# gongaa/Feedback-GNN

Measured on AMD Instinct MI355X. Metric: decoded codewords/sec, [[882,24]] 64-iter BP4 + feedback-GNN, higher is better.
Workload: dtype f32

## Files before the change

feedback_gnn_amd/csrc/fgnn_bp4.hip:

```cpp

#include <type_traits>

#include "fgnn_internal.h"
#include "fgnn_math.h"
#include "fgnn_math_ranged.h"
#include "fgnn_cn.h"

#ifndef FGNN_BP4_WAVES
#define FGNN_BP4_WAVES 7
#endif
#ifndef FGNN_HWT_PIN_CLIP_POINTS
#define FGNN_HWT_PIN_CLIP_POINTS 1
#endif
#ifndef FGNN_PHI_STAGE
#define FGNN_PHI_STAGE 1
#endif

namespace {

struct BpArgs {
    int B, num_iter, tpc, cpb, lds_per_cw, lch_off;
    float factor, llr_const;
    const float* llr_ch;
    const uint8_t* synd_x;
// ... 46 lines not shown
    {
        const float y = exp(-FG_MIN(FG_ABS(a - b), 20.0f));
        return log(1.0f + y);
    }
    static __device__ __forceinline__ float lse2(float a, float b)
    {
        return lse2_corr(a, b) + FG_MAX(a, b);
    }
    static __device__ __forceinline__ float phi(float x)
    {
        const float xc = FG_CLAMP(x, FG_PHI_MIN, FG_PHI_MAX);
        const float y = exp(xc);
        const float sp = (xc > FG_SOFTPLUS_THRESH) ? xc : log(1.0f + y);
        float r = sp - log(y - 1.0f);
#if FGNN_HWT_PIN_CLIP_POINTS
        r = (x >= FG_PHI_MAX) ? 0.0f : r;
        r = (x <= FG_PHI_MIN) ? 16.6355324f : r;
#endif
        return r;
    }
};

template <bool HWT = false>
__device__ __forceinline__ float logit_row_opt(const float* llr, const int* __restrict__ col, int deg, float phi0, bool shortcut)
{
    if (shortcut) {
        unsigned neg = 0;
        bool sat = true;
        for (int j = 0; j < deg; ++j) {
            const float v = llr[col[j]];
            neg ^= (v < 0.0f);
            sat = sat && (FG_ABS(v) >= FG_PHI_MAX);
        }
        if (__all(sat)) return with_sign(phi0, neg);
    }
    return logit_row<Mx<HWT>>(llr, col, deg);
}

template <int N, bool HWT = false>
__device__ __forceinline__ void phi_n(const float (&x)[N], float (&out)[N])
{
    if constexpr (HWT) {
#pragma unroll
        for (int k = 0; k < N; ++k) out[k] = Mx<true>::phi(x[k]);
        return;
    }
    const float* tab = fg_log_tab();
    float xc[N], y[N];
    uint32_t eb1[N], eb2[N], j1[N], j2[N];
#pragma unroll
    for (int k = 0; k < N; ++k) {
        xc[k] = FG_CLAMP(x[k], FG_PHI_MIN, FG_PHI_MAX);
        y[k] = fg_exp(xc[k]);
        const uint32_t w1 = fg_f2u(1.0f + y[k]) - FG_LOG_OFFS;
        const uint32_t w2 = fg_f2u(y[k] - 1.0f) - FG_LOG_OFFS;
        eb1[k] = w1 & 0xff800000u;
        eb2[k] = w2 & 0xff800000u;
        j1[k] = (w1 >> 18) & 31u;
        j2[k] = (w2 >> 18) & 31u;
    }
    __builtin_amdgcn_sched_barrier(0);
    float rc1[N], lc1[N], rc2[N], lc2[N];
#pragma unroll
    for (int k = 0; k < N; ++k) {
        rc1[k] = tab[j1[k]];
        lc1[k] = tab[32 + j1[k]];
        rc2[k] = tab[j2[k]];
        lc2[k] = tab[32 + j2[k]];
    }
    __builtin_amdgcn_sched_barrier(0);
#pragma unroll
    for (int k = 0; k < N; ++k) {
        const float a = fg_u2f(fg_f2u(rc1[k]) - eb1[k]);
        const float r1 = FG_FMA(y[k], a, a - 1.0f);
        float sp = FG_FMA((float)(int32_t)eb1[k], FG_LN2_S23, lc1[k] + fg_log1p_small(r1));
        sp = (xc[k] > FG_SOFTPLUS_THRESH) ? xc[k] : sp;
        const float mm = fg_u2f(fg_f2u(y[k] - 1.0f) - eb2[k]);
        const float r2 = FG_FMA(mm, rc2[k], -1.0f);
        const float lg = FG_FMA((float)(int32_t)eb2[k], FG_LN2_S23, lc2[k] + fg_log1p_small(r2));
        out[k] = sp - lg;
    }
}

template <int DC, bool HWT = false, bool F1 = false>
__device__ __forceinline__ bool cn_phi_regular(float* msg, const int (&sl)[DC], uint32_t neg0, float factor, float phi0,
                                               bool shortcut)
{
    constexpr int H = (DC % FGNN_PHI_STAGE == 0) ? FGNN_PHI_STAGE : DC / 2;
    static_assert(DC % H == 0, "a phi stage must take a whole fraction of a check");
    float v[DC], aa[DC];
    uint32_t neg = neg0;
    bool sat = true;
#pragma unroll
    for (int j = 0; j < DC; ++j) {
        v[j] = slot_ref(msg, sl[j]);
        neg ^= fg_f2u(v[j]);
        sat = sat && (FG_ABS(v[j]) >= FG_PHI_MAX);
    }
    if (shortcut && __all(sat)) {
#pragma unroll
        for (int j = 0; j < DC; ++j) {
            const float o = fg_u2f(fg_f2u(phi0) | ((neg ^ fg_f2u(v[j])) & 0x80000000u));
            slot_ref(msg, sl[j]) = F1 ? o : o * factor;
        }
        return true;
    }
#pragma unroll
    for (int g0 = 0; g0 < DC; g0 += H) {
        float xa[H], oa[H];
#pragma unroll
        for (int j = 0; j < H; ++j) xa[j] = FG_ABS(v[g0 + j]);
        phi_n<H, HWT>(xa, oa);
#pragma unroll
        for (int j = 0; j < H; ++j) aa[g0 + j] = oa[j];
    }
    float T = 0.0f;
#pragma unroll
    for (int j = 0; j < DC; ++j) T = T + aa[j];
#pragma unroll
    for (int g0 = 0; g0 < DC; g0 += H) {
        float xa[H], oa[H];
#pragma unroll
        for (int j = 0; j < H; ++j) xa[j] = T - aa[g0 + j];
        phi_n<H, HWT>(xa, oa);
#pragma unroll
        for (int j = 0; j < H; ++j) {
            const float o = fg_u2f(fg_f2u(oa[j]) | ((neg ^ fg_f2u(v[g0 + j])) & 0x80000000u));
            slot_ref(msg, sl[g0 + j]) = F1 ? o : o * factor;
        }
    }
    return false;
}

template <int DC>
__device__ __forceinline__ void cn_tanh_regular(float* msg, const int (&sl)[DC], unsigned synd, float factor)
{
    float t[DC];
    float P = 1.0f;
#pragma unroll
    for (int j = 0; j < DC; ++j) {
        float tj = fg_tanh(slot_ref(msg, sl[j]) / 2.0f);
        tj = (tj == 0.0f) ? 1e-12f : tj;
        P = (j == 0) ? tj : P * tj;
        t[j] = tj;
    }
    P = P * (synd ? -1.0f : 1.0f);
    const float clipv = 0.99999988f;
#pragma unroll
    for (int j = 0; j < DC; ++j) {
        float q = fg_rcp_unit(t[j]) * P;
        q = (FG_ABS(q) < 1e-7f) ? 0.0f : q;
        q = FG_MIN(FG_MAX(q, -clipv), clipv);
        slot_ref(msg, sl[j]) = (2.0f * fg_atanh(q)) * factor;
    }
}

template <bool HWT = false>
__device__ __forceinline__ bool cn_phi_generic(float* msg, const int* __restrict__ slot, int deg, unsigned synd, float factor,
                                               float phi0, bool shortcut)
{
    if (shortcut) {
        unsigned neg = synd;
        bool sat = true;
        for (int j = 0; j < deg; ++j) {
            const float v = msg[slot[j]];
            neg ^= (v < 0.0f);
            sat = sat && (FG_ABS(v) >= FG_PHI_MAX);
        }
        if (__all(sat)) {
            for (int j = 0; j < deg; ++j) {
                const int s = slot[j];
                msg[s] = with_sign(phi0, neg ^ (unsigned)(msg[s] < 0.0f)) * factor;
            }
            return true;
        }
    }
    cn_update<FGNN_CN_BOXPLUS_PHI, Mx<HWT>>(msg, slot, deg, synd, factor);
    return false;
}

__device__ __forceinline__ float softplus_saturated(float t)
{
    const float y = fg_exp(FG_MIN(FG_MAX(t, -87.0f), 0.0f));
    return (t > 0.0f) ? t : ((t < -87.0f) ? 0.0f : y);
}

template <int CN_TYPE, int DVX, int DVZ, int DC, bool OPT, bool HWT = false, int NQ = 0, bool TRACE = false, bool GMEM = false, int LSE = 2,
          int NT = 0>
__global__ void __launch_bounds__(1024) __attribute__((amdgpu_waves_per_eu(NQ > 0 ? FGNN_BP4_WAVES - 1 : FGNN_BP4_WAVES)))
bp4_kernel(GraphDev g, BpArgs a)
{
    static_assert(!(HWT && OPT), "the hardware-transcendental variant is the fixed dataflow only: the exact shortcuts are proofs about fgnn_math.h");
    static_assert(!GMEM || (DVX == 0 && !OPT && !HWT && NQ == 0 && !TRACE), "the global-memory variant is the plain runtime-degree kernel");
    using MX = Mx<HWT>;
    FG_LOG_TAB_SETUP();
    constexpr bool REGULAR = DVX > 0;
    constexpr bool LREG = NQ > 0;
    constexpr int NQA = LREG ? NQ : 1;
    static_assert(NT == 0 || (DVX > 0 && CN_TYPE == FGNN_CN_BOXPLUS_PHI && !LREG && !TRACE && !GMEM), "compile-time trips: the regular phi kernel");
    constexpr int CT = LREG ? NQ : NT;
    const int tpc = NT > 0 ? 256 : a.tpc;
    const bool opt_shortcut = OPT && a.shortcut != 0;
    const bool opt_exit = OPT && a.early_exit != 0;
    const bool shl = LSE == 2 ? a.shared_lse != 0 : LSE == 1;
    extern __shared__ float lds[];
    const int cwl = NT > 0 ? 0 : threadIdx.x / tpc;
    const int lane = threadIdx.x - cwl * tpc;
    const int slot_b = NT > 0 ? blockIdx.x : blockIdx.x * a.cpb + cwl;
    const bool active = slot_b < a.B;
    const int b = (active && a.index) ? a.index[slot_b] : slot_b;
    float* msg;
    if constexpr (GMEM) msg = a.gmem + (size_t)slot_b * a.lds_per_cw;
    else if constexpr (NT > 0) msg = lds;
    else msg = lds + (size_t)cwl * a.lds_per_cw;
    float* Lch = msg + a.lch_off;
    const int n = g.n;

    constexpr bool CLOSED_OK = REGULAR && CN_TYPE == FGNN_CN_BOXPLUS_PHI && !LREG && !TRACE;
    const bool zero_start = REGULAR && !TRACE && !a.msg_init_x && !a.msg_init_z && a.num_iter > 0;
    const bool first_closed = CLOSED_OK && zero_start && !a.llr_ch;
    const bool first_peeled = zero_start && a.llr_ch != nullptr;
    const bool fill = !first_closed && !first_peeled;
    if (active) {
        if (fill) {
            for (int e = lane; e < g.E_x; e += tpc) msg[e] = a.msg_init_x ? a.msg_init_x[(size_t)b * g.E_x + e] : 0.0f;
            for (int e = lane; e < g.E_z; e += tpc)
                msg[g.E_x + e] = a.msg_init_z ? a.msg_init_z[(size_t)b * g.E_z + e] : 0.0f;
        }
        if (a.llr_ch && !LREG)
            for (int i = lane; i < 3 * n; i += tpc) Lch[i] = a.llr_ch[(size_t)b * 3 * n + i];
    }
    float lreg[3][NQA];
    if constexpr (LREG) {
#pragma unroll
        for (int i = 0; i < NQ; ++i) {
            const int v = lane + i * tpc;
            const bool in = active && v < n;
#pragma unroll
            for (int c = 0; c < 3; ++c) lreg[c][i] = in ? a.llr_ch[(size_t)b * 3 * n + c * n + v] : 0.0f;
        }
    }
    if (fill || (a.llr_ch && !LREG)) __syncthreads();

    const uint8_t* sx = a.synd_x + (size_t)b * g.m_x;
    const uint8_t* sz = a.synd_z + (size_t)b * g.m_z;
    const int lane_c = lane + (tpc >> 1) < tpc ? lane + (tpc >> 1) : lane - tpc + (tpc >> 1);

    const float phi0 = MX::phi(0.0f);
    (void)phi0;
    unsigned* sigw = reinterpret_cast<unsigned*>(msg + a.sig_off);
    int* flags = reinterpret_cast<int*>(sigw + n);
    bool a1 = false, a2 = false;
    if (opt_exit) {
        for (int v = lane; v < n; v += tpc) sigw[v] = fill ? 0xffffffffu : 0u;
        if (lane < 4) flags[lane] = 0;
        __syncthreads();
    }
    int it_begin = 0;
    if constexpr (CLOSED_OK) {
        if (first_closed) {
            const float L = a.llr_const;
            const float Y = (0.0f + 0.0f) + L, X = 0.0f + L, Z = 0.0f + L;
            const float nu_x = MX::softplus(-X) - MX::lse2(-(Z - 0.0f), -(Y - 0.0f));
            const float nu_z = MX::softplus(-Z) - MX::lse2(-(X - 0.0f), -(Y - 0.0f));
            if (active)
                for (int c = lane_c; c < g.m; c += tpc) {
                    const unsigned synd = (c < g.m_x ? sx[c] : sz[c - g.m_x]) & 1u;
                    const uint4 pk = reinterpret_cast<const uint4*>(g.cslot16)[c];
                    const unsigned w[4] = {pk.x, pk.y, pk.z, pk.w};
                    const float nu = c < g.m_x ? nu_x : nu_z;
                    const unsigned ng = nu < 0.0f;
                    unsigned neg = synd;
                    const float aa = MX::phi(FG_ABS(nu));
                    float T = 0.0f;
#pragma unroll
                    for (int j = 0; j < DC; ++j) {
                        neg ^= ng;
                        T = T + aa;
                    }
                    const float val = with_sign(MX::phi(T - aa), neg ^ ng) * a.factor;
#pragma unroll
                    for (int j = 0; j < DC; ++j) slot_ref(msg, (int)((w[j >> 1] >> ((j & 1) * 16)) & 0xffffu)) = val;
                }
            if (opt_exit) a1 = FG_ABS(nu_x) >= FG_PHI_MAX && FG_ABS(nu_z) >= FG_PHI_MAX;
            it_begin = 1;
            __syncthreads();
        }
    }
    const bool cn_one = a.cpb == 1, cn_f1 = a.factor == 1.0f;
    unsigned synd_bits = 0;
    if (active) {
        int i = 0;
        for (int c = lane_c; c < g.m && i < 32; c += tpc, ++i) synd_bits |= ((c < g.m_x ? sx[c] : sz[c - g.m_x]) & 1u) << i;
    }
    const bool synd_in_reg = (g.m + tpc - 1) / tpc <= 32;
    unsigned row_off = 16u * (unsigned)lane_c;
    auto trace_step = [&](const int k) __attribute__((always_inline)) {
        float* tlx = msg + a.trace_off;
        float* tlz = tlx + n;
        if (active && a.tape_x) {
            float* px = a.tape_x + ((size_t)k * a.B + b) * g.E_x;
            float* pz = a.tape_z + ((size_t)k * a.B + b) * g.E_z;
            for (int e = lane; e < g.E_x; e += tpc) px[e] = msg[e];
            for (int e = lane; e < g.E_z; e += tpc) pz[e] = msg[g.E_x + e];
        }
        if (active)
            for (int v = lane; v < n; v += tpc) {
                const int x0 = g.vptr_x[v], x1 = g.vptr_x[v + 1], z0 = g.vptr_z[v], z1 = g.vptr_z[v + 1];
                float Sz = 0.0f, Sx = 0.0f;
                for (int e = z0; e < z1; ++e) Sz = Sz + msg[e];
                for (int e = x0; e < x1; ++e) Sx = Sx + msg[e];
                const float lx = a.llr_ch ? Lch[v] : a.llr_const, ly = a.llr_ch ? Lch[n + v] : a.llr_const,
                            lz = a.llr_ch ? Lch[2 * n + v] : a.llr_const;
                const float Y = (Sz + Sx) + ly;
                const float X = Sz + lx;
                const float Z = Sx + lz;
                tlz[v] = MX::softplus(-X) - MX::lse2(-Z, -Y);
                tlx[v] = MX::softplus(-Z) - MX::lse2(-X, -Y);
            }
        __syncthreads();
        if (active) {
            float* tx = a.trace_x + ((size_t)k * a.B + b) * g.rows[0];
            for (int r = lane; r < g.rows[0]; r += tpc) {
                const int p0 = g.rptr[0][r];
                tx[r] = logit_row<Mx<HWT>>(tlx, g.rcol[0] + p0, g.rptr[0][r + 1] - p0);
            }
            float* tz = a.trace_z + ((size_t)k * a.B + b) * g.rows[1];
            for (int r = lane; r < g.rows[1]; r += tpc) {
                const int p0 = g.rptr[1][r];
                tz[r] = logit_row<Mx<HWT>>(tlz, g.rcol[1] + p0, g.rptr[1][r + 1] - p0);
            }
        }
    };
    if constexpr (TRACE) trace_step(0);
    if constexpr (REGULAR && !TRACE) {
        if (first_peeled && active) {
            auto vn_first = [&](const int v, const float lx, const float ly, const float lz) __attribute__((always_inline)) {
                const float Y = (0.0f + 0.0f) + ly;
                const float X = 0.0f + lx;
                const float Z = 0.0f + lz;
                const float numx = MX::softplus(-X);
                const float numz = MX::softplus(-Z);
                const float Ze = Z - 0.0f, Xe = X - 0.0f, Ye = Y - 0.0f;
                float ox, oz;
                if (shl) {
                    ox = numx - (MX::lse2_corr(-Z, -Y) + FG_MAX(-Ze, -Ye));
                    oz = numz - (MX::lse2_corr(-X, -Y) + FG_MAX(-Xe, -Ye));
                } else {
                    ox = numx - MX::lse2(-Ze, -Ye);
                    oz = numz - MX::lse2(-Xe, -Ye);
                }
                float* px = msg + v * DVX;
                float* pz = msg + g.E_x + v * DVZ;
#pragma unroll
                for (int k = 0; k < DVX; ++k) px[k] = ox;
#pragma unroll
                for (int k = 0; k < DVZ; ++k) pz[k] = oz;
            };
            if constexpr (LREG) {
#pragma unroll
                for (int i = 0; i < NQ; ++i) {
                    const int v = lane + i * tpc;
                    if (v < n) vn_first(v, lreg[0][i], lreg[1][i], lreg[2][i]);
                }
            } else {
                for (int v = lane; v < n; v += tpc) vn_first(v, Lch[v], Lch[n + v], Lch[2 * n + v]);
            }
        }
    }
    for (int it = it_begin; it < a.num_iter; ++it) {
        bool changed = false, cn_slow = false;
        auto vn_body = [&](const int v, const float lx, const float ly, const float lz) __attribute__((always_inline)) {
                if constexpr (REGULAR) {
                    float* px = msg + v * DVX;
                    float* pz = msg + g.E_x + v * DVZ;
                    float mx[DVX], mz[DVZ];
                    float Sz = 0.0f, Sx = 0.0f;
#pragma unroll
                    for (int k = 0; k < DVZ; ++k) { mz[k] = pz[k]; Sz = Sz + mz[k]; }
// ... 81 lines not shown
                            sig |= sign_bit(mm) << (e - x0);
                        }
                        for (int e = z0; e < z1; ++e) {
                            const float mm = msg[e];
                            sat = sat && (shl || FG_ABS((X - mm) - (Y - mm)) >= 20.0f);
                            sig |= sign_bit(mm) << ((x1 - x0) + (e - z0));
                        }
                        if (opt_exit && sigw[v] != sig) {
                            changed = true;
                            sigw[v] = sig;
                        }
                        if (__all(sat)) {
                            const float nx = softplus_saturated(-X), nz = softplus_saturated(-Z);
                            for (int e = x0; e < x1; ++e) {
                                const float mm = msg[e];
                                const float Ze = Z - mm, Ye = Y - mm;
                                msg[e] = nx - (0.0f + FG_MAX(-Ze, -Ye));
                            }
                            for (int e = z0; e < z1; ++e) {
                                const float mm = msg[e];
                                const float Xe = X - mm, Ye = Y - mm;
                                msg[e] = nz - (0.0f + FG_MAX(-Xe, -Ye));
                            }
                            return;
                        }
                    }
                    const float numx = MX::softplus(-X);
                    const float numz = MX::softplus(-Z);
                    if (shl) {
                        const float cx = MX::lse2_corr(-Z, -Y), cz = MX::lse2_corr(-X, -Y);
                        for (int e = x0; e < x1; ++e) {
                            float m = msg[e];
                            float Ze = Z - m, Ye = Y - m;
                            msg[e] = numx - (cx + FG_MAX(-Ze, -Ye));
                        }
                        for (int e = z0; e < z1; ++e) {
                            float m = msg[e];
                            float Xe = X - m, Ye = Y - m;
                            msg[e] = numz - (cz + FG_MAX(-Xe, -Ye));
                        }
                        return;
                    }
                    for (int e = x0; e < x1; ++e) {
                        float m = msg[e];
                        float Ze = Z - m, Ye = Y - m;
                        msg[e] = numx - MX::lse2(-Ze, -Ye);
                    }
                    for (int e = z0; e < z1; ++e) {
                        float m = msg[e];
                        float Xe = X - m, Ye = Y - m;
                        msg[e] = numz - MX::lse2(-Xe, -Ye);
                    }
                }
            };
        if (active && !(first_peeled && it == 0)) {
            if constexpr (LREG) {
#pragma unroll
                for (int i = 0; i < NQ; ++i) {
                    const int v = lane + i * tpc;
                    if (v < n) vn_body(v, lreg[0][i], lreg[1][i], lreg[2][i]);
                }
            } else if constexpr (NT > 0) {
#pragma unroll
                for (int i = 0; i < NT; ++i) {
                    const int v = lane + i * 256;
                    if (i + 1 < NT || v < n) vn_body(v, a.llr_const, a.llr_const, a.llr_const);
                }
            } else {
                for (int v = lane; v < n; v += tpc) {
                    if (a.llr_ch) vn_body(v, Lch[v], Lch[n + v], Lch[2 * n + v]);
                    else vn_body(v, a.llr_const, a.llr_const, a.llr_const);
                }
            }
        }
        if (opt_exit && changed) flags[2 * (it & 1)] = 1;
        __syncthreads();
        if (opt_exit && lane == 0) {
            flags[2 * ((it + 1) & 1)] = 0;
            flags[2 * ((it + 1) & 1) + 1] = 0;
        }
        if constexpr (REGULAR && CT > 0 && CN_TYPE == FGNN_CN_BOXPLUS_PHI) {
            auto cn_trips = [&](auto f1) __attribute__((always_inline)) {
                constexpr bool F1 = decltype(f1)::value;
                const char* rows = reinterpret_cast<const char*>(g.cslot16);
#pragma unroll
                for (int i = 0; i < CT; ++i) {
                    const bool in = (!LREG && i + 1 < CT) || lane_c + i * tpc < g.m;
                    if (in) {
                        const char* base = rows + (size_t)i * (size_t)(16u * (unsigned)tpc);
                        asm volatile("" : "+v"(row_off));
                        if constexpr (NT > 0) asm volatile("" : "+s"(base));
                        typedef unsigned Row __attribute__((ext_vector_type(4)));
                        const Row pk = *(const __attribute__((address_space(1))) Row*)(base + row_off);
                        const unsigned w[4] = {pk.x, pk.y, pk.z, pk.w};
                        int sl[DC];
#pragma unroll
                        for (int j = 0; j < DC; ++j) sl[j] = (int)((w[j >> 1] >> ((j & 1) * 16)) & 0xffffu);
                        const bool fast = cn_phi_regular<DC, HWT, F1>(lds, sl, synd_bits << (31 - i), F1 ? 1.0f : a.factor, phi0, opt_shortcut);
                        cn_slow = !fast || cn_slow;
                    }
                }
            };
            if (active) {
                if (cn_f1) cn_trips(std::true_type{});
                else cn_trips(std::false_type{});
            }
        } else if (active) {
            int ci = 0;
            for (int c = lane_c; c < g.m; c += tpc, ++ci) {
                const unsigned synd = synd_in_reg ? (synd_bits >> ci) & 1u : (c < g.m_x ? sx[c] : sz[c - g.m_x]) & 1u;
                if constexpr (REGULAR) {
                    const uint4 pk = reinterpret_cast<const uint4*>(g.cslot16)[c];
                    const unsigned w[4] = {pk.x, pk.y, pk.z, pk.w};
                    int sl[DC];
#pragma unroll
                    for (int j = 0; j < DC; ++j) sl[j] = (int)((w[j >> 1] >> ((j & 1) * 16)) & 0xffffu);
                    if constexpr (CN_TYPE == FGNN_CN_BOXPLUS_PHI) {
                        bool fast;
                        if (cn_one && cn_f1) fast = cn_phi_regular<DC, HWT, true>(lds, sl, synd << 31, 1.0f, phi0, opt_shortcut);
                        else if (cn_one) fast = cn_phi_regular<DC, HWT, false>(lds, sl, synd << 31, a.factor, phi0, opt_shortcut);
                        else fast = cn_phi_regular<DC, HWT, false>(msg, sl, synd << 31, a.factor, phi0, opt_shortcut);
                        cn_slow = !fast || cn_slow;
                    } else if constexpr (CN_TYPE == FGNN_CN_MINSUM) {
                        cn_minsum_regular<DC>(msg, sl, DC, synd, a.factor);
                    } else {
                        cn_tanh_regular<DC>(msg, sl, synd, a.factor);
                    }
                } else {
                    const int c0 = g.cptr[c], deg = g.cptr[c + 1] - c0;
                    if constexpr (CN_TYPE == FGNN_CN_BOXPLUS_PHI)
                        cn_slow = !cn_phi_generic<HWT>(msg, g.cslot + c0, deg, synd, a.factor, phi0, opt_shortcut) || cn_slow;
                    else cn_update<CN_TYPE, Mx<HWT>>(msg, g.cslot + c0, deg, synd, a.factor);
                }
            }
        }
        if (opt_exit && cn_slow) flags[2 * (it & 1) + 1] = 1;
        __syncthreads();
        if (opt_exit) {
            const bool stable = a1 && a2 && flags[2 * (it & 1)] == 0;
            a2 = a1;
            a1 = flags[2 * (it & 1) + 1] == 0;
            if (stable) break;
        }
        if constexpr (TRACE) trace_step(it + 1);
    }

    if (active) {
        if (a.msg_out_x)
            for (int e = lane; e < g.E_x; e += tpc) a.msg_out_x[(size_t)b * g.E_x + e] = msg[e];
        if (a.msg_out_z)
            for (int e = lane; e < g.E_z; e += tpc) a.msg_out_z[(size_t)b * g.E_z + e] = msg[g.E_x + e];
    }
    auto total_body = [&](const int v, const float lx, const float ly, const float lz) __attribute__((always_inline)) {
            const int x0 = g.vptr_x[v], x1 = g.vptr_x[v + 1], z0 = g.vptr_z[v], z1 = g.vptr_z[v + 1];
            float Sz = 0.0f, Sx = 0.0f;
            for (int e = z0; e < z1; ++e) Sz = Sz + msg[e];
            for (int e = x0; e < x1; ++e) Sx = Sx + msg[e];
            const float Y = (Sz + Sx) + ly;
            const float X = Sz + lx;
            const float Z = Sx + lz;
            float* o = a.llr_out + (size_t)b * 3 * n;
            o[v] = X;
            o[n + v] = Y;
            o[2 * n + v] = Z;
            int d = 0;
            float best = 0.0f;
            if (X < best) { best = X; d = 1; }
            if (Z < best) { best = Z; d = 2; }
            if (Y < best) { best = Y; d = 3; }
            a.x_hat[(size_t)b * n + v] = (uint8_t)(d & 1);
            a.z_hat[(size_t)b * n + v] = (uint8_t)(d >> 1);
    };
    if (active) {
        if constexpr (LREG) {
#pragma unroll
            for (int i = 0; i < NQ; ++i) {
                const int v = lane + i * tpc;
                if (v < n) total_body(v, lreg[0][i], lreg[1][i], lreg[2][i]);
            }
        } else {
            for (int v = lane; v < n; v += tpc) {
                if (a.llr_ch) total_body(v, Lch[v], Lch[n + v], Lch[2 * n + v]);
                else total_body(v, a.llr_const, a.llr_const, a.llr_const);
            }
        }
    }
    if (a.flagged) {
        uint8_t* dec = reinterpret_cast<uint8_t*>(msg + a.flag_off);
        unsigned* fword = reinterpret_cast<unsigned*>(dec + ((n + 3) & ~3));
        __syncthreads();
        if (active)
            for (int v = lane; v < n; v += tpc) {
                dec[v] = (uint8_t)(a.x_hat[(size_t)b * n + v] | (a.z_hat[(size_t)b * n + v] << 1));
            }
        if (lane == 0) *fword = 0u;
        __syncthreads();
        unsigned mine = 0;
        if (active)
            for (int c = lane; c < g.m; c += tpc) {
                const int sh = c < g.m_x ? 1 : 0;
                unsigned par = (c < g.m_x ? sx[c] : sz[c - g.m_x]) & 1u;
                for (int e = g.cptr[c]; e < g.cptr[c + 1]; ++e) par ^= (dec[g.cvn[e]] >> sh) & 1u;
                mine |= par;
            }
        if (mine) atomicOr(fword, 1u);
        __syncthreads();
        if (active && lane == 0) a.flagged[b] = (uint8_t)(*fword != 0u);
    }
    if (!a.x_logit && !a.z_logit) return;
    __syncthreads();
    float* llx = msg;
    float* llz = msg + n;
    if (active)
        for (int v = lane; v < n; v += tpc) {
            const float* o = a.llr_out + (size_t)b * 3 * n;
            const float X = o[v], Y = o[n + v], Z = o[2 * n + v];
            const bool sat = opt_shortcut && FG_ABS(X) > FG_SOFTPLUS_THRESH && FG_ABS(Z) > FG_SOFTPLUS_THRESH &&
                             FG_ABS((-Z) - (-Y)) >= 20.0f && FG_ABS((-X) - (-Y)) >= 20.0f;
            if (opt_shortcut && __all(sat)) {
                llz[v] = softplus_saturated(-X) - (0.0f + FG_MAX(-Z, -Y));
                llx[v] = softplus_saturated(-Z) - (0.0f + FG_MAX(-X, -Y));
                continue;
            }
            llz[v] = MX::softplus(-X) - MX::lse2(-Z, -Y);
            llx[v] = MX::softplus(-Z) - MX::lse2(-X, -Y);
        }
    __syncthreads();
    if (active) {
        if (a.x_logit)
            for (int r = lane; r < g.rows[0]; r += tpc) {
                const int p0 = g.rptr[0][r];
                a.x_logit[(size_t)b * g.rows[0] + r] = logit_row_opt<HWT>(llx, g.rcol[0] + p0, g.rptr[0][r + 1] - p0, phi0, opt_shortcut);
            }
        if (a.z_logit)
            for (int r = lane; r < g.rows[1]; r += tpc) {
                const int p0 = g.rptr[1][r];
                a.z_logit[(size_t)b * g.rows[1] + r] = logit_row_opt<HWT>(llz, g.rcol[1] + p0, g.rptr[1][r + 1] - p0, phi0, opt_shortcut);
            }
    }
}

using Bp4Kernel = void (*)(GraphDev, BpArgs);

template <int NQ, bool OPT, int LSE, int NT = 0>
constexpr Bp4Kernel bp4_lse_kernel = bp4_kernel<FGNN_CN_BOXPLUS_PHI, 3, 3, 6, OPT, false, NQ, false, false, LSE, NT>;
constexpr Bp4Kernel bp4_lse_kernels[3][2][2] = {
    {{bp4_lse_kernel<0, false, 0>, bp4_lse_kernel<0, false, 1>}, {bp4_lse_kernel<0, true, 0>, bp4_lse_kernel<0, true, 1>}},
    {{bp4_lse_kernel<4, false, 0>, bp4_lse_kernel<4, false, 1>}, {bp4_lse_kernel<4, true, 0>, bp4_lse_kernel<4, true, 1>}},
    {{bp4_lse_kernel<5, false, 0>, bp4_lse_kernel<5, false, 1>}, {bp4_lse_kernel<5, true, 0>, bp4_lse_kernel<5, true, 1>}}};

constexpr Bp4Kernel bp4_nt_kernels[2][2][2] = {
    {{bp4_lse_kernel<0, false, 0, 4>, bp4_lse_kernel<0, false, 1, 4>}, {bp4_lse_kernel<0, true, 0, 4>, bp4_lse_kernel<0, true, 1, 4>}},
    {{bp4_lse_kernel<0, false, 0, 5>, bp4_lse_kernel<0, false, 1, 5>}, {bp4_lse_kernel<0, true, 0, 5>, bp4_lse_kernel<0, true, 1, 5>}}};

template <int CN_TYPE, int DVX, int DVZ, int DC>
int launch_bp4_k(const fgnn_graph* g, const BpArgs& a, const LaunchGeom& L, size_t lds_bytes, hipStream_t st)
{
    Bp4Kernel kern = a.shortcut ? bp4_kernel<CN_TYPE, DVX, DVZ, DC, true> : bp4_kernel<CN_TYPE, DVX, DVZ, DC, false>;
    if constexpr ((DVX == 3 && DVZ == 3 && DC == 6) || DVX == 0) {
        if (a.trace_x) kern = bp4_kernel<CN_TYPE, DVX, DVZ, DC, false, false, 0, true>;
    }
    if constexpr (CN_TYPE == FGNN_CN_BOXPLUS_PHI) {
        if (a.hwt) kern = bp4_kernel<CN_TYPE, DVX, DVZ, DC, false, true>;
        if constexpr (DVX == 3 && DVZ == 3 && DC == 6) {
            if (!a.trace_x && !a.hwt) kern = bp4_lse_kernels[a.lreg ? a.lreg - 3 : 0][a.shortcut][a.shared_lse];
            if (!a.trace_x && !a.hwt && a.nt) kern = bp4_nt_kernels[a.nt - 4][a.shortcut][a.shared_lse];
        }
    }
    return fgnn_launch(kern, dim3(L.blocks), dim3(L.threads), lds_bytes, st, g->d, a);
}

struct Bp4Plan {
    size_t lds_bytes;
    bool gmem;
    size_t ws_bytes;
};

template <int CN_TYPE>
int launch_bp4(const fgnn_graph* g, const BpArgs& a, const LaunchGeom& L, const Bp4Plan& p, hipStream_t st)
{
    if (p.gmem)
        return fgnn_launch(bp4_kernel<CN_TYPE, 0, 0, 0, false, false, 0, false, true>, dim3(L.blocks), dim3(L.threads), 0, st, g->d, a);
    const GraphDev& d = g->d;
    if (d.cslot16 && !g->force_generic) {
        if (d.dvx == 3 && d.dvz == 3 && d.dc == 6) return launch_bp4_k<CN_TYPE, 3, 3, 6>(g, a, L, p.lds_bytes, st);
        if (d.dvx == 4 && d.dvz == 4 && d.dc == 8 && !a.trace_x) return launch_bp4_k<CN_TYPE, 4, 4, 8>(g, a, L, p.lds_bytes, st);
    }
    return launch_bp4_k<CN_TYPE, 0, 0, 0>(g, a, L, p.lds_bytes, st);
}

Bp4Plan plan_bp4(const fgnn_graph* g, int cn_type, const LaunchGeom& L, BpArgs& a, bool gmem = false)
{
    const GraphDev& d = g->d;
    const int n = d.n;
    const bool trace = a.trace_x != nullptr, phi = cn_type == FGNN_CN_BOXPLUS_PHI;
    auto round4 = [](int floats) { return (floats + 3) & ~3; };
    a.shared_lse = g->bp4_shared_lse ? 1 : 0;
    a.hwt = (g->hw_transcendentals && phi && !trace && !gmem) ? 1 : 0;
    a.shortcut = (g->shortcut && !a.hwt && !trace && !gmem) ? 1 : 0;
    a.lch_off = d.E > 2 * n ? d.E : 2 * n;
    const int per_thread = (n + L.tpc - 1) / L.tpc, per_thread_c = (d.m + L.tpc - 1) / L.tpc;
    const int trips = per_thread > per_thread_c ? per_thread : per_thread_c;
    const bool r336 = d.cslot16 && !g->force_generic && d.dvx == 3 && d.dvz == 3 && d.dc == 6;
    const bool fixed_trips = !trace && !a.hwt && !gmem && phi && L.cpb == 1 && r336;
    a.lreg = (a.llr_ch && fixed_trips && trips <= 5) ? (trips <= 4 ? 4 : 5) : 0;
    a.nt = (!a.llr_ch && fixed_trips && L.tpc == 256 && per_thread == per_thread_c && (trips == 4 || trips == 5)) ? trips : 0;
    int per = a.lch_off + ((a.llr_ch && !a.lreg) ? 3 * n : 0);
    a.trace_off = 0;
    if (trace) {
        a.trace_off = per;
        per += 2 * n;
    }
    if (!gmem) per = round4(per);
    a.sig_off = per;
    int tail = 0;
    a.early_exit = (a.shortcut && g->early_exit && d.max_vdeg <= 32 && phi && L.cpb == 1 && a.num_iter > 2) ? 1 : 0;
    if (a.early_exit) {
        if (((size_t)per * L.cpb + n + 4) * sizeof(float) <= FGNN_LDS_BUDGET) tail += n + 4;
        else a.early_exit = 0;
    }
    a.flag_off = 0;
    if (a.flagged) {
        const int need = round4(n) / 4 + 1;
        if (a.lch_off >= 2 * n + need) {
            a.flag_off = 2 * n;
        } else {
            a.flag_off = per + tail;
            tail += need;
        }
    }
    if (gmem) {
        a.lds_per_cw = round4(per + tail);
        return {0, true, (size_t)L.blocks * (size_t)a.lds_per_cw * sizeof(float)};
    }
    a.lds_per_cw = per;
    const size_t lds_bytes = ((size_t)per * L.cpb + tail) * sizeof(float);
    if (lds_bytes > FGNN_LDS_BUDGET) return plan_bp4(g, cn_type, L, a, true);
    return {lds_bytes, false, 0};
}

}

static int bp4_decode_core(const fgnn_graph* g, int cn_type, int num_iter, float normalization_factor, const float* llr_ch,
                           float llr_const, const uint8_t* synd_x, const uint8_t* synd_z, int B, const float* msg_init_x,
                           const float* msg_init_z, float* llr_out, uint8_t* x_hat, uint8_t* z_hat, float* x_logit,
                           float* z_logit, float* msg_out_x, float* msg_out_z, const int* index, uint8_t* flagged,
                           float* trace_x, float* trace_z, float* tape_x, float* tape_z, void* stream)
{
    if (!g) return fgnn_fail(FGNN_ERR_ARG, "graph is NULL");
    if (B < 0 || num_iter < 0) return fgnn_fail(FGNN_ERR_ARG, "B and num_iter must be >= 0");
    if (cn_type < 0 || cn_type > 2) return fgnn_fail(FGNN_ERR_ARG, "Unknown node type.");
    if ((x_logit && !g->d.rptr[0]) || (z_logit && !g->d.rptr[1]))
        return fgnn_fail(FGNN_ERR_STATE, "logit row sets not installed (fgnn_graph_set_rows)");
    if (B == 0) return FGNN_OK;
    if (!synd_x || !synd_z || !llr_out || !x_hat || !z_hat) return fgnn_fail(FGNN_ERR_ARG, "required buffer is NULL");
    FGNN_DEVICE_GUARD(g->device);
    const LaunchGeom L = fgnn_geom(g, B);
    if (flagged && L.cpb != 1) return fgnn_fail(FGNN_ERR_STATE, "the fused flag test needs one codeword per workgroup");
    BpArgs a;
    a.B = B;
    a.num_iter = num_iter;
    a.tpc = L.tpc;
    a.cpb = L.cpb;
    a.factor = normalization_factor;
    a.llr_const = llr_const;
    a.llr_ch = llr_ch;
    a.synd_x = synd_x;
    a.synd_z = synd_z;
    a.msg_init_x = msg_init_x;
    a.msg_init_z = msg_init_z;
    a.llr_out = llr_out;
    a.x_hat = x_hat;
    a.z_hat = z_hat;
    a.x_logit = x_logit;
    a.z_logit = z_logit;
    a.msg_out_x = msg_out_x;
    a.msg_out_z = msg_out_z;
    a.index = index;
    a.flagged = flagged;
    a.gmem = nullptr;
    a.trace_x = trace_x;
    a.trace_z = trace_z;
    a.tape_x = tape_x;
    a.tape_z = tape_z;
    const Bp4Plan p = plan_bp4(g, cn_type, L, a);
    hipStream_t st = static_cast<hipStream_t>(stream);
    if (p.gmem) {
        if (trace_x) return fgnn_fail(FGNN_ERR_ARG, "code too large for the LDS-resident trace kernel");
        if (L.cpb != 1) return fgnn_fail(FGNN_ERR_STATE, "the global-memory BP4 variant needs one codeword per workgroup");
// ... 62 lines not shown
```

feedback_gnn_amd/csrc/fgnn_graph.hip:

```cpp
#include <algorithm>
#include <cstring>
#include <numeric>

#include "fgnn_internal.h"

static thread_local std::string g_err;
void fgnn_set_error(const std::string& s) { g_err = s; }
int fgnn_fail(int code, const std::string& s)
{
    g_err = s;
    return code;
}
extern "C" const char* fgnn_last_error(void) { return g_err.c_str(); }
extern "C" int fgnn_version(void) { return 2; }

namespace {

template <typename T>
int upload(fgnn_graph* g, const std::vector<T>& h, const T** dst)
{
    void* p = nullptr;
    size_t bytes = std::max<size_t>(h.size(), 1) * sizeof(T);
    FGNN_HIP_CHECK(hipMalloc(&p, bytes));
    g->allocs.push_back(p);
// ... 62 lines not shown

extern "C" int fgnn_graph_create(int n, int m_x, int m_z, int nnz_x, const int32_t* chk_x, const int32_t* var_x,
                                 int nnz_z, const int32_t* chk_z, const int32_t* var_z, int device, fgnn_graph** out)
{
    if (!out) return fgnn_fail(FGNN_ERR_ARG, "out is NULL");
    if (n <= 0 || m_x <= 0 || m_z <= 0 || nnz_x <= 0 || nnz_z <= 0)
        return fgnn_fail(FGNN_ERR_ARG, "n, m_x, m_z and the edge counts must be positive");
    const int32_t* chk[2] = {chk_x, chk_z};
    const int32_t* var[2] = {var_x, var_z};
    const int nnz[2] = {nnz_x, nnz_z};
    const int m[2] = {m_x, m_z};
    for (int s = 0; s < 2; ++s)
        for (int i = 0; i < nnz[s]; ++i)
            if (chk[s][i] < 0 || chk[s][i] >= m[s] || var[s][i] < 0 || var[s][i] >= n)
                return fgnn_fail(FGNN_ERR_ARG, "edge index out of range");
    FGNN_DEVICE_GUARD(device);
    fgnn_graph* g = new fgnn_graph();
    std::memset(&g->d, 0, sizeof(g->d));
    std::memset(g->row_alloc, 0, sizeof(g->row_alloc));
    g->device = device;
    g->user_launch = false;
    GraphDev& d = g->d;
    d.n = n;
    d.m_x = m_x;
    d.m_z = m_z;
    d.m = m_x + m_z;
    d.E_x = nnz_x;
    d.E_z = nnz_z;
    d.E = nnz_x + nnz_z;

    std::vector<int> vptr[2], vchk_side[2];
    for (int s = 0; s < 2; ++s) {
        coo_to_csr(n, nnz[s], var[s], chk[s], vptr[s], vchk_side[s]);
        for (int v = 0; v < n; ++v)
            for (int e = vptr[s][v]; e + 1 < vptr[s][v + 1]; ++e)
                if (vchk_side[s][e] == vchk_side[s][e + 1]) {
                    delete g;
                    return fgnn_fail(FGNN_ERR_ARG, "duplicate edge");
                }
        g->h_chk[s] = std::vector<int32_t>(vchk_side[s].begin(), vchk_side[s].end());
        g->h_var[s].resize(nnz[s]);
        for (int v = 0; v < n; ++v)
            for (int e = vptr[s][v]; e < vptr[s][v + 1]; ++e) g->h_var[s][e] = v;
    }
    std::vector<int> vptr_x = vptr[0], vptr_z = vptr[1], vchk(d.E);
    for (auto& x : vptr_z) x += d.E_x;
    std::copy(vchk_side[0].begin(), vchk_side[0].end(), vchk.begin());
    std::copy(vchk_side[1].begin(), vchk_side[1].end(), vchk.begin() + d.E_x);
    std::vector<int> cptr(d.m + 1, 0), cslot(d.E), cvn(d.E);
    {
        std::vector<int> deg(d.m, 0);
        for (int s = 0; s < 2; ++s)
            for (int i = 0; i < nnz[s]; ++i) deg[(s ? m_x : 0) + chk[s][i]]++;
        for (int c = 0; c < d.m; ++c) cptr[c + 1] = cptr[c] + deg[c];
        std::vector<int> fill(d.m, 0);
        for (int s = 0; s < 2; ++s)
            for (int v = 0; v < n; ++v)
                for (int e = vptr[s][v]; e < vptr[s][v + 1]; ++e) {
                    int c = (s ? m_x : 0) + vchk_side[s][e];
                    int pos = cptr[c] + fill[c]++;
                    cslot[pos] = e + (s ? d.E_x : 0);
                    cvn[pos] = v;
                }
    }
    d.dvx = uniform_degree(vptr[0]);
    d.dvz = uniform_degree(vptr[1]);
    d.dc = uniform_degree(cptr);
    d.max_vdeg = 0;
    for (int v = 0; v < n; ++v)
        d.max_vdeg = std::max(d.max_vdeg, (vptr[0][v + 1] - vptr[0][v]) + (vptr[1][v + 1] - vptr[1][v]));
    d.max_cdeg = d.max_cdeg_x = 0;
    for (int c = 0; c < d.m; ++c) {
        d.max_cdeg = std::max(d.max_cdeg, cptr[c + 1] - cptr[c]);
        if (c < m_x) d.max_cdeg_x = std::max(d.max_cdeg_x, cptr[c + 1] - cptr[c]);
    }
    int rc;
    if (d.dvx > 0 && d.dvz > 0 && d.dc > 0 && d.dc <= 8 && (long long)d.E * 4 < 65536) {
        std::vector<uint16_t> pk((size_t)d.m * 8, 0);
        for (int c = 0; c < d.m; ++c)
            for (int j = 0; j < d.dc; ++j) pk[(size_t)c * 8 + j] = (uint16_t)(4 * cslot[cptr[c] + j]);
        if ((rc = upload(g, pk, &d.cslot16))) {
            fgnn_graph_destroy(g);
            return rc;
        }
    }
    if ((rc = upload(g, vptr_x, &d.vptr_x)) || (rc = upload(g, vptr_z, &d.vptr_z)) || (rc = upload(g, vchk, &d.vchk)) ||
        (rc = upload(g, cptr, &d.cptr)) || (rc = upload(g, cslot, &d.cslot)) || (rc = upload(g, cvn, &d.cvn))) {
        fgnn_graph_destroy(g);
        return rc;
    }
    default_launch(g);
    *out = g;
    return FGNN_OK;
}

extern "C" void fgnn_graph_destroy(fgnn_graph* g)
{
    if (!g) return;
    fgnn_device_guard _dg(g->device);
    for (hipEvent_t e : g->prof_ev) (void)hipEventDestroy(e);
    for (void* p : g->basis_dev)
        if (p) (void)hipFree(p);
    for (void* p : g->allocs) (void)hipFree(p);
    for (auto& r : g->row_alloc)
        for (void* p : r)
            if (p) (void)hipFree(p);
    delete g;
}

extern "C" int fgnn_graph_set_rows(fgnn_graph* g, int which, int rows, int nnz, const int32_t* row, const int32_t* col)
{
    if (!g || which < 0 || which > 5 || rows < 0 || nnz < 0) return fgnn_fail(FGNN_ERR_ARG, "bad row-set arguments");
    for (int i = 0; i < nnz; ++i)
        if (row[i] < 0 || row[i] >= rows || col[i] < 0 || col[i] >= g->d.n)
            return fgnn_fail(FGNN_ERR_ARG, "row-set index out of range");
    FGNN_DEVICE_GUARD(g->device);
    std::vector<int> ptr, c;
    coo_to_csr(rows, nnz, row, col, ptr, c);
    for (void*& p : g->row_alloc[which])
        if (p) {
            (void)hipFree(p);
            p = nullptr;
        }
    void *dp = nullptr, *dc = nullptr;
    FGNN_HIP_CHECK(hipMalloc(&dp, ptr.size() * sizeof(int)));
    g->row_alloc[which][0] = dp;
    FGNN_HIP_CHECK(hipMalloc(&dc, std::max<size_t>(c.size(), 1) * sizeof(int)));
    g->row_alloc[which][1] = dc;
    FGNN_HIP_CHECK(hipMemcpy(dp, ptr.data(), ptr.size() * sizeof(int), hipMemcpyHostToDevice));
    if (!c.empty()) FGNN_HIP_CHECK(hipMemcpy(dc, c.data(), c.size() * sizeof(int), hipMemcpyHostToDevice));
    g->d.rows[which] = rows;
    g->d.rptr[which] = static_cast<const int*>(dp);
    g->d.rcol[which] = static_cast<const int*>(dc);
    if (which < 2) {
        const int n = g->d.n;
        std::vector<int> tp(n + 1, 0), tr(std::max<size_t>(c.size(), 1), 0);
        for (int x : c) tp[x + 1]++;
        for (int v = 0; v < n; ++v) tp[v + 1] += tp[v];
        std::vector<int> fill(tp.begin(), tp.end() - 1);
        for (int r = 0; r < rows; ++r)
            for (int p = ptr[r]; p < ptr[r + 1]; ++p) tr[fill[c[p]]++] = r;
        void *tpd = nullptr, *trd = nullptr;
        FGNN_HIP_CHECK(hipMalloc(&tpd, tp.size() * sizeof(int)));
        g->row_alloc[which][2] = tpd;
        FGNN_HIP_CHECK(hipMalloc(&trd, tr.size() * sizeof(int)));
        g->row_alloc[which][3] = trd;
        FGNN_HIP_CHECK(hipMemcpy(tpd, tp.data(), tp.size() * sizeof(int), hipMemcpyHostToDevice));
        FGNN_HIP_CHECK(hipMemcpy(trd, tr.data(), tr.size() * sizeof(int), hipMemcpyHostToDevice));
        g->d.tptr[which] = static_cast<const int*>(tpd);
        g->d.trow[which] = static_cast<const int*>(trd);
    }
    return FGNN_OK;
}

extern "C" int fgnn_graph_set_launch(fgnn_graph* g, int threads_per_codeword, int codewords_per_block)
{
    if (!g) return fgnn_fail(FGNN_ERR_ARG, "graph is NULL");
    if (threads_per_codeword <= 0 && codewords_per_block <= 0) {
        default_launch(g);
        g->user_launch = false;
        return FGNN_OK;
    }
    int tpc = threads_per_codeword > 0 ? threads_per_codeword : g->tpc;
    int cpb = codewords_per_block > 0 ? codewords_per_block : 1;
    if (tpc * cpb > 1024 || (tpc * cpb) % 64 != 0)
        return fgnn_fail(FGNN_ERR_ARG, "threads_per_codeword*codewords_per_block must be a multiple of 64 and <= 1024");
// ... 92 lines not shown
```

feedback_gnn_amd/csrc/fgnn_internal.h:

```cpp
#pragma once
#include <hip/hip_runtime.h>
#include <stdint.h>
#include <string>
#include <vector>

#include "../../include/fgnn.h"

struct GraphDev {
    int n, m_x, m_z, m, E_x, E_z, E;
    const int* vptr_x;
    const int* vptr_z;
    const int* vchk;
    const int* cptr;
    const int* cslot;
    const int* cvn;
    const uint16_t* cslot16;
    int rows[6];
    const int* rptr[6];
    const int* rcol[6];
    const int* tptr[2];
    const int* trow[2];
    int dvx, dvz, dc;
    int max_vdeg;
    int max_cdeg, max_cdeg_x;
};

struct fgnn_graph {
    GraphDev d;
    int device;
    int tpc, cpb;
    bool user_launch;
    bool shortcut = true;
    bool early_exit = true;
    bool hw_transcendentals = false;
    bool bp4_shared_lse = false;
    int gnn_stream = 1;
    bool gnn_factored = false;
    bool force_generic = false;
    std::vector<void*> allocs;
    std::vector<int32_t> h_chk[2], h_var[2];
    void* row_alloc[6][4];
    void* basis_dev[2] = {nullptr, nullptr};
    int basis_rank[2] = {0, 0};
    mutable bool prof_on = false;
    mutable int prof_n = 0;
    mutable std::vector<hipEvent_t> prof_ev;
    mutable std::vector<int> prof_iters, prof_batch;
};

#if defined(__HIPCC__)
typedef const float __attribute__((address_space(4)))* scalar_fp;
__device__ __forceinline__ scalar_fp as_scalar(const float* p) { return (scalar_fp)(unsigned long long)p; }
#endif

struct WeightsDev {
    const float* w1t[2];
    const float* b1[2];
    const float* w2[2];
    const float* b2[2];
    const float* wet;
    const float* be;
    const float* wout;
    const float* bout;
    const float* lane_tab;
    const float* msg_rows[2];
    const float* emb_rows;
    const float* emb_quads;
};

constexpr int FGNN_GEN_MAX_LAYERS = 12;
constexpr int FGNN_GEN_MAX_D = 32, FGNN_GEN_MAX_W = 96;
struct GnnGeneralDev {
    int D, H, L, reduce_op, act, bias, nl;
    int K[FGNN_GEN_MAX_LAYERS], J[FGNN_GEN_MAX_LAYERS], act_l[FGNN_GEN_MAX_LAYERS];
    const float* W[FGNN_GEN_MAX_LAYERS];
    const float* b[FGNN_GEN_MAX_LAYERS];
};

struct fgnn_weights {
    WeightsDev d;
    int device;
    void* blob;
    bool general = false;
    GnnGeneralDev gen;
};

struct fgnn_gnnbp4_train_view {
    int device, D, H, L, reduce_op, act, bias, use_attributes;
    const float* W[7][4];
    const float* b[7][4];
    int K[7][4], J[7][4];
    const float* winv;
    const float* binv;
};
bool fgnn_gnnbp4_weights_train_view(const fgnn_gnnbp4_weights* w, fgnn_gnnbp4_train_view* out);

void fgnn_set_error(const std::string& s);
int fgnn_fail(int code, const std::string& s);
#define FGNN_HIP_CHECK(expr)                                                                          \
    do {                                                                                              \
        hipError_t _e = (expr);                                                                       \
        if (_e != hipSuccess)                                                                         \
            return fgnn_fail(FGNN_ERR_HIP, std::string(#expr) + ": " + hipGetErrorString(_e));        \
    } while (0)

struct fgnn_device_guard {
    int prev = -1;
    hipError_t err = hipSuccess;
    explicit fgnn_device_guard(int device)
    {
        err = hipGetDevice(&prev);
        if (err == hipSuccess && prev != device) err = hipSetDevice(device);
        else prev = -1;
    }
    ~fgnn_device_guard()
    {
        if (prev >= 0) (void)hipSetDevice(prev);
    }
    fgnn_device_guard(const fgnn_device_guard&) = delete;
    fgnn_device_guard& operator=(const fgnn_device_guard&) = delete;
};
#define FGNN_DEVICE_GUARD(device)                                                                     \
    fgnn_device_guard _dev_guard(device);                                                             \
    if (_dev_guard.err != hipSuccess)                                                                 \
        return fgnn_fail(FGNN_ERR_HIP, std::string("hipSetDevice: ") + hipGetErrorString(_dev_guard.err))

template <typename W>
int fgnn_weights_upload(W* w, const std::vector<float>& h, const char* what)
{
    w->blob = nullptr;
    hipError_t e = hipMalloc(&w->blob, h.size() * sizeof(float));
    if (e == hipSuccess) e = hipMemcpy(w->blob, h.data(), h.size() * sizeof(float), hipMemcpyHostToDevice);
    if (e != hipSuccess) {
        if (w->blob) (void)hipFree(w->blob);
        delete w;
        return fgnn_fail(FGNN_ERR_HIP, std::string(what) + hipGetErrorString(e));
    }
    return FGNN_OK;
}

template <typename W>
void fgnn_weights_free(W* w)
{
    if (!w) return;
    fgnn_device_guard _dg(w->device);
    if (w->blob) (void)hipFree(w->blob);
    delete w;
}

constexpr int FGNN_PROF_TAG_GNN = -1;
constexpr int FGNN_PROF_TAG_GNNBP4 = -2;
struct fgnn_prof_scope {
    const fgnn_graph* g;
    hipStream_t st;
    bool on;
    fgnn_prof_scope(const fgnn_graph* g_, hipStream_t st_) : g(g_), st(st_)
    {
        on = g->prof_on && (size_t)(2 * g->prof_n + 1) < g->prof_ev.size();
        if (on && hipEventRecord(g->prof_ev[2 * g->prof_n], st) != hipSuccess) on = false;
    }
    void done(int tag, int B)
    {
        if (!on) return;
        if (hipEventRecord(g->prof_ev[2 * g->prof_n + 1], st) != hipSuccess) return;
        g->prof_iters[g->prof_n] = tag;
        g->prof_batch[g->prof_n] = B;
        g->prof_n++;
    }
};

constexpr size_t FGNN_LDS_BUDGET = 160 * 1024 - 256;

template <typename... Params, typename... Args>
int fgnn_launch(void (*kern)(Params...), dim3 grid, dim3 block, size_t lds, hipStream_t st, Args... args)
{
    if (lds > 48 * 1024)
        FGNN_HIP_CHECK(hipFuncSetAttribute(reinterpret_cast<const void*>(kern), hipFuncAttributeMaxDynamicSharedMemorySize, (int)lds));
    hipLaunchKernelGGL(kern, grid, block, lds, st, args...);
    FGNN_HIP_CHECK(hipGetLastError());
    return FGNN_OK;
}

struct LaunchGeom {
    int tpc, cpb, threads, blocks;
};
LaunchGeom fgnn_geom(const fgnn_graph* g, int B);

int fgnn_bp4_decode_impl(const fgnn_graph* g, int cn_type, int num_iter, float normalization_factor, const float* llr_ch,
                         float llr_const, const uint8_t* synd_x, const uint8_t* synd_z, int B, const float* msg_init_x,
                         const float* msg_init_z, float* llr_out, uint8_t* x_hat, uint8_t* z_hat, float* x_logit,
                         float* z_logit, float* msg_out_x, float* msg_out_z, const int* index, uint8_t* flagged, void* stream);
int fgnn_feedback_gnn_impl(const fgnn_graph* g, const fgnn_weights* w, const float* llr, const float* logit_hx,
                           const float* logit_hz, const uint8_t* synd_x, const uint8_t* synd_z, int B, float* out,
                           const int* index, void* stream);
int fgnn_flag_update_impl(const fgnn_graph* g, const uint8_t* x_hat, const uint8_t* z_hat, const uint8_t* synd_x,
                          const uint8_t* synd_z, int B, uint8_t* errors, const int* index, void* stream);
int fgnn_merge_impl(const uint8_t* errors, const uint8_t* x_upd, const uint8_t* z_upd, int B, int n, uint8_t* x_hat, uint8_t* z_hat,
                    const int* index, void* stream);
```

Measured before the change: 972,000.

## Precompute absolute LDS byte addresses per check row and add fixed-trip lreg5 kernel

Adds a 32-bit per-check slot table whose entries already hold absolute LDS byte addresses, offset past the static log table. The phi check-node update then loads and stores through raw address-space-3 pointers instead of unpacking 16-bit indices and adding the msg base. This removes the shift/mask and address arithmetic per slot. It also routes the lreg=5 case with tpc 256 to a new compile-time-trip kernel variant. In exchange each row fetch grows from 16 to 24 bytes of global memory, and correctness now depends on the static LDS size matching the assumed offset, which a runtime check enforces.

```diff
diff --git a/feedback_gnn_amd/csrc/fgnn_bp4.hip b/feedback_gnn_amd/csrc/fgnn_bp4.hip
--- a/feedback_gnn_amd/csrc/fgnn_bp4.hip
+++ b/feedback_gnn_amd/csrc/fgnn_bp4.hip
@@ -152,10 +152,19 @@
     }
 }
 
-template <int DC, bool HWT = false, bool F1 = false>
+template <int DC, bool HWT = false, bool F1 = false, bool ABS = false>
 __device__ __forceinline__ bool cn_phi_regular(float* msg, const int (&sl)[DC], uint32_t neg0, float factor, float phi0,
                                                bool shortcut)
 {
+    typedef __attribute__((address_space(3))) float lds_float;
+    auto ld = [&](const int s) __attribute__((always_inline)) {
+        if constexpr (ABS) return *reinterpret_cast<lds_float*>((uintptr_t)(unsigned)s);
+        else return slot_ref(msg, s);
+    };
+    auto st = [&](const int s, const float x) __attribute__((always_inline)) {
+        if constexpr (ABS) *reinterpret_cast<lds_float*>((uintptr_t)(unsigned)s) = x;
+        else slot_ref(msg, s) = x;
+    };
     constexpr int H = (DC % FGNN_PHI_STAGE == 0) ? FGNN_PHI_STAGE : DC / 2;
     static_assert(DC % H == 0, "a phi stage must take a whole fraction of a check");
     float v[DC], aa[DC];
@@ -163,7 +172,7 @@
     bool sat = true;
 #pragma unroll
     for (int j = 0; j < DC; ++j) {
-        v[j] = slot_ref(msg, sl[j]);
+        v[j] = ld(sl[j]);
         neg ^= fg_f2u(v[j]);
         sat = sat && (FG_ABS(v[j]) >= FG_PHI_MAX);
     }
@@ -171,7 +180,7 @@
 #pragma unroll
         for (int j = 0; j < DC; ++j) {
             const float o = fg_u2f(fg_f2u(phi0) | ((neg ^ fg_f2u(v[j])) & 0x80000000u));
-            slot_ref(msg, sl[j]) = F1 ? o : o * factor;
+            st(sl[j], F1 ? o : o * factor);
         }
         return true;
     }
@@ -196,7 +205,7 @@
 #pragma unroll
         for (int j = 0; j < H; ++j) {
             const float o = fg_u2f(fg_f2u(oa[j]) | ((neg ^ fg_f2u(v[g0 + j])) & 0x80000000u));
-            slot_ref(msg, sl[g0 + j]) = F1 ? o : o * factor;
+            st(sl[g0 + j], F1 ? o : o * factor);
         }
     }
     return false;
@@ -257,7 +266,7 @@
 
 template <int CN_TYPE, int DVX, int DVZ, int DC, bool OPT, bool HWT = false, int NQ = 0, bool TRACE = false, bool GMEM = false, int LSE = 2,
           int NT = 0>
-__global__ void __launch_bounds__(1024) __attribute__((amdgpu_waves_per_eu(NQ > 0 ? FGNN_BP4_WAVES - 1 : FGNN_BP4_WAVES)))
+__global__ void __launch_bounds__(1024) __attribute__((amdgpu_waves_per_eu(NQ > 0 && NT == 0 ? FGNN_BP4_WAVES - 1 : FGNN_BP4_WAVES)))
 bp4_kernel(GraphDev g, BpArgs a)
 {
     static_assert(!(HWT && OPT), "the hardware-transcendental variant is the fixed dataflow only: the exact shortcuts are proofs about fgnn_math.h");
@@ -267,7 +276,7 @@
     constexpr bool REGULAR = DVX > 0;
     constexpr bool LREG = NQ > 0;
     constexpr int NQA = LREG ? NQ : 1;
-    static_assert(NT == 0 || (DVX > 0 && CN_TYPE == FGNN_CN_BOXPLUS_PHI && !LREG && !TRACE && !GMEM), "compile-time trips: the regular phi kernel");
+    static_assert(NT == 0 || (DVX > 0 && CN_TYPE == FGNN_CN_BOXPLUS_PHI && (!LREG || (NT == NQ && NQ == 5)) && !TRACE && !GMEM), "compile-time trips: the regular phi kernel");
     constexpr int CT = LREG ? NQ : NT;
     const int tpc = NT > 0 ? 256 : a.tpc;
     const bool opt_shortcut = OPT && a.shortcut != 0;
@@ -364,7 +373,7 @@
         for (int c = lane_c; c < g.m && i < 32; c += tpc, ++i) synd_bits |= ((c < g.m_x ? sx[c] : sz[c - g.m_x]) & 1u) << i;
     }
     const bool synd_in_reg = (g.m + tpc - 1) / tpc <= 32;
-    unsigned row_off = 16u * (unsigned)lane_c;
+    unsigned row_off = 32u * (unsigned)lane_c;
     auto trace_step = [&](const int k) __attribute__((always_inline)) {
         float* tlx = msg + a.trace_off;
         float* tlz = tlx + n;
@@ -612,21 +621,21 @@
         if constexpr (REGULAR && CT > 0 && CN_TYPE == FGNN_CN_BOXPLUS_PHI) {
             auto cn_trips = [&](auto f1) __attribute__((always_inline)) {
                 constexpr bool F1 = decltype(f1)::value;
-                const char* rows = reinterpret_cast<const char*>(g.cslot16);
+                const char* rows = reinterpret_cast<const char*>(g.cslot32);
 #pragma unroll
                 for (int i = 0; i < CT; ++i) {
                     const bool in = (!LREG && i + 1 < CT) || lane_c + i * tpc < g.m;
                     if (in) {
-                        const char* base = rows + (size_t)i * (size_t)(16u * (unsigned)tpc);
+                        const char* base = rows + (size_t)i * (size_t)(32u * (unsigned)tpc);
                         asm volatile("" : "+v"(row_off));
                         if constexpr (NT > 0) asm volatile("" : "+s"(base));
-                        typedef unsigned Row __attribute__((ext_vector_type(4)));
-                        const Row pk = *(const __attribute__((address_space(1))) Row*)(base + row_off);
-                        const unsigned w[4] = {pk.x, pk.y, pk.z, pk.w};
-                        int sl[DC];
-#pragma unroll
-                        for (int j = 0; j < DC; ++j) sl[j] = (int)((w[j >> 1] >> ((j & 1) * 16)) & 0xffffu);
-                        const bool fast = cn_phi_regular<DC, HWT, F1>(lds, sl, synd_bits << (31 - i), F1 ? 1.0f : a.factor, phi0, opt_shortcut);
+                        typedef unsigned Row4 __attribute__((ext_vector_type(4)));
+                        typedef unsigned Row2 __attribute__((ext_vector_type(2)));
+                        const Row4 pa = *(const __attribute__((address_space(1))) Row4*)(base + row_off);
+                        const Row2 pb = *(const __attribute__((address_space(1))) Row2*)(base + row_off + 16);
+                        static_assert(DC == 6, "a row of g.cslot32 holds six slots");
+                        const int sl[DC] = {(int)pa.x, (int)pa.y, (int)pa.z, (int)pa.w, (int)pb.x, (int)pb.y};
+                        const bool fast = cn_phi_regular<DC, HWT, F1, true>(lds, sl, synd_bits << (31 - i), F1 ? 1.0f : a.factor, phi0, opt_shortcut);
                         cn_slow = !fast || cn_slow;
                     }
                 }
@@ -779,10 +788,39 @@
     {{bp4_lse_kernel<4, false, 0>, bp4_lse_kernel<4, false, 1>}, {bp4_lse_kernel<4, true, 0>, bp4_lse_kernel<4, true, 1>}},
     {{bp4_lse_kernel<5, false, 0>, bp4_lse_kernel<5, false, 1>}, {bp4_lse_kernel<5, true, 0>, bp4_lse_kernel<5, true, 1>}}};
 
+constexpr Bp4Kernel bp4_lreg5_nt_kernels[2][2] = {
+    {bp4_lse_kernel<5, false, 0, 5>, bp4_lse_kernel<5, false, 1, 5>}, {bp4_lse_kernel<5, true, 0, 5>, bp4_lse_kernel<5, true, 1, 5>}};
+
 constexpr Bp4Kernel bp4_nt_kernels[2][2][2] = {
     {{bp4_lse_kernel<0, false, 0, 4>, bp4_lse_kernel<0, false, 1, 4>}, {bp4_lse_kernel<0, true, 0, 4>, bp4_lse_kernel<0, true, 1, 4>}},
     {{bp4_lse_kernel<0, false, 0, 5>, bp4_lse_kernel<0, false, 1, 5>}, {bp4_lse_kernel<0, true, 0, 5>, bp4_lse_kernel<0, true, 1, 5>}}};
 
+int bp4_check_lds_base()
+{
+    static const int rc = [] {
+        auto check = [](Bp4Kernel k) {
+            hipFuncAttributes fa;
+            if (hipFuncGetAttributes(&fa, reinterpret_cast<const void*>(k)) != hipSuccess) return 1;
+            return fa.sharedSizeBytes == FGNN_LDS_STATIC_BYTES ? 0 : 2;
+        };
+        for (const auto& by_opt : bp4_nt_kernels)
+            for (const auto& by_lse : by_opt)
+                for (Bp4Kernel k : by_lse)
+                    if (const int e = check(k)) return e;
+        for (const auto& by_lse : bp4_lreg5_nt_kernels)
+            for (Bp4Kernel k : by_lse)
+                if (const int e = check(k)) return e;
+        for (int q = 1; q < 3; ++q)
+            for (const auto& by_lse : bp4_lse_kernels[q])
+                for (Bp4Kernel k : by_lse)
+                    if (const int e = check(k)) return e;
+        return 0;
+    }();
+    if (rc == 1) return fgnn_fail(FGNN_ERR_HIP, "hipFuncGetAttributes failed for a BP4 kernel");
+    if (rc == 2) return fgnn_fail(FGNN_ERR_STATE, "a fixed-trip BP4 kernel's static LDS is not the log table alone: g.cslot32 would address the wrong slots");
+    return FGNN_OK;
+}
+
 template <int CN_TYPE, int DVX, int DVZ, int DC>
 int launch_bp4_k(const fgnn_graph* g, const BpArgs& a, const LaunchGeom& L, size_t lds_bytes, hipStream_t st)
 {
@@ -793,8 +831,11 @@
     if constexpr (CN_TYPE == FGNN_CN_BOXPLUS_PHI) {
         if (a.hwt) kern = bp4_kernel<CN_TYPE, DVX, DVZ, DC, false, true>;
         if constexpr (DVX == 3 && DVZ == 3 && DC == 6) {
+            if (!a.trace_x && !a.hwt && (a.lreg || a.nt))
+                if (const int rc = bp4_check_lds_base()) return rc;
             if (!a.trace_x && !a.hwt) kern = bp4_lse_kernels[a.lreg ? a.lreg - 3 : 0][a.shortcut][a.shared_lse];
-            if (!a.trace_x && !a.hwt && a.nt) kern = bp4_nt_kernels[a.nt - 4][a.shortcut][a.shared_lse];
+            if (!a.trace_x && !a.hwt && a.nt)
+                kern = a.lreg ? bp4_lreg5_nt_kernels[a.shortcut][a.shared_lse] : bp4_nt_kernels[a.nt - 4][a.shortcut][a.shared_lse];
         }
     }
     return fgnn_launch(kern, dim3(L.blocks), dim3(L.threads), lds_bytes, st, g->d, a);
@@ -831,10 +872,11 @@
     a.lch_off = d.E > 2 * n ? d.E : 2 * n;
     const int per_thread = (n + L.tpc - 1) / L.tpc, per_thread_c = (d.m + L.tpc - 1) / L.tpc;
     const int trips = per_thread > per_thread_c ? per_thread : per_thread_c;
-    const bool r336 = d.cslot16 && !g->force_generic && d.dvx == 3 && d.dvz == 3 && d.dc == 6;
+    const bool r336 = d.cslot16 && d.cslot32 && !g->force_generic && d.dvx == 3 && d.dvz == 3 && d.dc == 6;
     const bool fixed_trips = !trace && !a.hwt && !gmem && phi && L.cpb == 1 && r336;
     a.lreg = (a.llr_ch && fixed_trips && trips <= 5) ? (trips <= 4 ? 4 : 5) : 0;
     a.nt = (!a.llr_ch && fixed_trips && L.tpc == 256 && per_thread == per_thread_c && (trips == 4 || trips == 5)) ? trips : 0;
+    if (a.lreg == 5 && L.tpc == 256) a.nt = 5;
     int per = a.lch_off + ((a.llr_ch && !a.lreg) ? 3 * n : 0);
     a.trace_off = 0;
     if (trace) {
diff --git a/feedback_gnn_amd/csrc/fgnn_graph.hip b/feedback_gnn_amd/csrc/fgnn_graph.hip
--- a/feedback_gnn_amd/csrc/fgnn_graph.hip
+++ b/feedback_gnn_amd/csrc/fgnn_graph.hip
@@ -168,6 +168,15 @@
         if ((rc = upload(g, pk, &d.cslot16))) {
             fgnn_graph_destroy(g);
             return rc;
+        }
+        if (d.dvx == 3 && d.dvz == 3 && d.dc == 6) {
+            std::vector<uint32_t> pw((size_t)d.m * 8, 0);
+            for (int c = 0; c < d.m; ++c)
+                for (int j = 0; j < d.dc; ++j) pw[(size_t)c * 8 + j] = (uint32_t)FGNN_LDS_STATIC_BYTES + pk[(size_t)c * 8 + j];
+            if ((rc = upload(g, pw, &d.cslot32))) {
+                fgnn_graph_destroy(g);
+                return rc;
+            }
         }
     }
     if ((rc = upload(g, vptr_x, &d.vptr_x)) || (rc = upload(g, vptr_z, &d.vptr_z)) || (rc = upload(g, vchk, &d.vchk)) ||
diff --git a/feedback_gnn_amd/csrc/fgnn_internal.h b/feedback_gnn_amd/csrc/fgnn_internal.h
--- a/feedback_gnn_amd/csrc/fgnn_internal.h
+++ b/feedback_gnn_amd/csrc/fgnn_internal.h
@@ -15,6 +15,7 @@
     const int* cslot;
     const int* cvn;
     const uint16_t* cslot16;
+    const uint32_t* cslot32;
     int rows[6];
     const int* rptr[6];
     const int* rcol[6];
@@ -169,7 +170,8 @@
     }
 };
 
-constexpr size_t FGNN_LDS_BUDGET = 160 * 1024 - 256;
+constexpr size_t FGNN_LDS_STATIC_BYTES = 256;
+constexpr size_t FGNN_LDS_BUDGET = 160 * 1024 - FGNN_LDS_STATIC_BYTES;
 
 template <typename... Params, typename... Args>
 int fgnn_launch(void (*kern)(Params...), dim3 grid, dim3 block, size_t lds, hipStream_t st, Args... args)
```

Measured after the change: 981,800, median of 6. 1.0% higher.
